# utcsilab/score-based-channels

Measured on AMD Instinct MI355X. Metric: channels/s full ALD inference, CDL-C Nt64xNr16, higher is better.
Workload: dtype f16x2 (every fp32 operand as two fp16 terms of a power-of-two-scaled value = 22-bit significand, hh + hl + lh on the fp16 matrix cores, fp32 accumulate; fp32-class by the gate tests/test_gpu_parity.py::test_f16x2_is_fp32_class and held to every reference golden at the north_star tolerance; unconditi

## Files before the change

score_based_channels_amd/csrc/conv_down.hip:

```cpp
#include <stdlib.h>
#include <string.h>
#include <type_traits>
#include "conv_common.h"

namespace sbc {

typedef float f32x4v __attribute__((ext_vector_type(4)));

struct DownParams {
    const float* __restrict__ a;
    const float* __restrict__ x;
    float* __restrict__ out;
    const float* __restrict__ stats;
    const uint4* __restrict__ w4;
    const uint4* __restrict__ w2;
    const float* __restrict__ bias;
    const float* __restrict__ bias2;
    unsigned* __restrict__ range_flag;
    float* __restrict__ calib;
    int B, H;
};

template <int B_, int E_, class F>
__device__ __forceinline__ void down_static_for(F&& f) {
    if constexpr (B_ < E_) {
        f(std::integral_constant<int, B_>{});
        down_static_for<B_ + 1, E_>(f);
    }
}

template <int CIN, int COUT, int W>
__global__ __launch_bounds__(256, 2) void conv_down_kernel(DownParams p) {
    constexpr int WO = W / 2, R = 8, NR = 2 * R + 2;
    constexpr int RP = W == 16 ? 12 : 6;
    constexpr int CG = CIN / 8, KH = CIN / 32, C4 = CIN / 4, NCB = COUT / 16;
    constexpr int NU = R * WO / 16;
    constexpr int RPU = 16 / WO;
    constexpr int PS = (2 * NR * RP * 16 + 255) / 256 * 256;
    constexpr int TERM = CG * PS;
    static_assert(NCB == 4, "four waves, one 16-output-channel block each");
    static_assert((W == 16 && CIN == 32) || (W == 8 && CIN == 64), "res2.0 (32 -> 64 at 16-pixel rows) and res3.0 (64 -> 64 at 8)");
    extern __shared__ __attribute__((aligned(256))) unsigned char smem[];

    const int tid = threadIdx.x, lane = tid & 63;
    const int cb = __builtin_amdgcn_readfirstlane(tid >> 6);
    const int kq = lane >> 4, n = lane & 15;
    const int H = p.H, HO = H / 2;
    const int tiles = HO / R;
    const int s = blockIdx.x / tiles, y0 = (blockIdx.x - s * tiles) * R;
    const int r_in0 = 2 * y0 - 1;

    const int wl_base = (((kq >> 1) * (COUT / 32) + (cb >> 1)) * 2) * 64 + (16 * (cb & 1) + n) + 32 * (kq & 1);
    constexpr int WD = 4;
    uint4 wr[WD][2];
    auto ldw = [&](const uint4* __restrict__ w, int tap, int kh, int slot) {
        const int idx = wl_base + ((tap * (CIN / 16) + 2 * kh) * (COUT / 32) * 2) * 64;
        wr[slot][0] = w[idx];
        wr[slot][1] = w[idx + 64];
    };
    const float4 tr4 = f16x2_trailer(reinterpret_cast<const float4*>(p.w4), 16 * (CIN / 16) * (COUT / 32) * 2);
    const float4 tr2 = f16x2_trailer(reinterpret_cast<const float4*>(p.w2), 4 * (CIN / 16) * (COUT / 32) * 2);
    const float scale_m = __builtin_bit_cast(float, __builtin_amdgcn_readfirstlane(__builtin_bit_cast(int, tr4.x)));
    const float scale_s = __builtin_bit_cast(float, __builtin_amdgcn_readfirstlane(__builtin_bit_cast(int, tr2.x)));
    const float descale_m = tr4.y, descale_s = tr2.y;
    const bool elu_acc = __builtin_amdgcn_readfirstlane(__builtin_bit_cast(int, tr4.w)) != 0;
    unsigned rbits = 0;

    const int c4 = tid % C4;
    constexpr int CPR = W * C4;
    auto plane_dst = [&](int prow, int col) {
        return smem + (c4 >> 1) * PS + (((col & 1) * NR + prow) * RP + (col >> 1) + (col & 1)) * 16 + (c4 & 1) * 8;
    };
    for (int i = tid; i < 2 * TERM / 16; i += 256) *reinterpret_cast<uint4*>(smem + i * 16) = make_uint4(0, 0, 0, 0);

    constexpr int NQA = NR * CPR / 256, NQX = 2 * R * CPR / 256;
    static_assert(NR * CPR % 256 == 0 && 2 * R * CPR % 256 == 0, "whole rounds of chunks");
    float4 va[NQA];
    const float* a_base = p.a + (size_t)s * H * W * CIN;
#pragma unroll
    for (int k = 0; k < NQA; ++k) {
        const int q = k * 256 + tid, prow = q / CPR;
        const int r = r_in0 + prow;
        va[k] = make_float4(0.f, 0.f, 0.f, 0.f);
        if (r >= 0 && r < H) va[k] = *reinterpret_cast<const float4*>(a_base + (size_t)r * W * CIN + (q - prow * CPR) * 4);
    }
    const float* st = p.stats + (size_t)s * 3 * CIN + c4 * 4;
    const float4 mu = *reinterpret_cast<const float4*>(st), sc = *reinterpret_cast<const float4*>(st + CIN),
                 sh = *reinterpret_cast<const float4*>(st + 2 * CIN);
    ldw(p.w4, 0, 0, 0);
    ldw(p.w4, 1 / KH, 1 % KH, 1);
    ldw(p.w4, 2 / KH, 2 % KH, 2);
    __syncthreads();
    float ta = 0.f;
#pragma unroll
    for (int k = 0; k < NQA; ++k) {
        const int q = k * 256 + tid, prow = q / CPR, col = (q - prow * CPR) / C4;
        const int r = r_in0 + prow;
        if (r < 0 || r >= H) continue;
        float4 v = va[k];
        v.x = fmaf(v.x - mu.x, sc.x, sh.x); v.y = fmaf(v.y - mu.y, sc.y, sh.y);
        v.z = fmaf(v.z - mu.z, sc.z, sh.z); v.w = fmaf(v.w - mu.w, sc.w, sh.w);
        v = elu4(v, elu_acc);
        StageScale ss{scale_m, ta};
        scale_track(v, &ss);
        ta = ss.amax;
        uint2 h, l;
        split_f16x2(v, scale_m, h, l);
        unsigned char* dst = plane_dst(prow, col);
        *reinterpret_cast<uint2*>(dst) = h;
        *reinterpret_cast<uint2*>(dst + TERM) = l;
    }
    pair_range_tile(ta, scale_m, rbits, p.calib);
    float4 vx[NQX];
    const float* x_base = p.x + ((size_t)s * H + 2 * y0) * W * CIN;
#pragma unroll
    for (int k = 0; k < NQX; ++k) vx[k] = *reinterpret_cast<const float4*>(x_base + (size_t)(k * 256 + tid) * 4);
    lds_barrier();

    const int yl0 = n / WO, xo = n % WO;
    const int rd_base = kq * PS + ((2 * yl0) * RP + xo) * 16;
    f32x4v accm[NU], accs[NU];
    auto kloop = [&](auto mainc, const uint4* __restrict__ w, f32x4v* acc) {
        constexpr bool MAIN = decltype(mainc)::value;
        constexpr int KT = MAIN ? 4 : 2, NS = KT * KT * KH;
        down_static_for<0, NS>([&](auto sc_) {
            constexpr int s_ = decltype(sc_)::value;
            constexpr int tap = s_ / KH, kh = s_ % KH, tp = tap / KT, tq = tap % KT;
            if constexpr (s_ + WD - 1 < NS) ldw(w, (s_ + WD - 1) / KH, (s_ + WD - 1) % KH, (s_ + WD - 1) % WD);
            const f16x8 wh = __builtin_bit_cast(f16x8, wr[s_ % WD][0]);
            const f16x8 wl = __builtin_bit_cast(f16x8, wr[s_ % WD][1]);
            constexpr int prow = MAIN ? tp : tp + 1, q = MAIN ? tq : tq + 1;
            constexpr int off = (4 * kh) * PS + ((((q + 1) & 1) * NR + prow) * RP + (q >> 1)) * 16;
            f16x8 xh[NU], xl[NU];
#pragma unroll
            for (int u = 0; u < NU; ++u) {
                xh[u] = *reinterpret_cast<const f16x8*>(smem + rd_base + off + (2 * u * RPU * RP) * 16);
                xl[u] = *reinterpret_cast<const f16x8*>(smem + rd_base + off + (2 * u * RPU * RP) * 16 + TERM);
            }
#pragma unroll
            for (int u = 0; u < NU; ++u) {
                const f32x4v z = s_ == 0 ? f32x4v{0.f, 0.f, 0.f, 0.f} : acc[u];
                acc[u] = __builtin_amdgcn_mfma_f32_16x16x32_f16(wh, xl[u], z, 0, 0, 0);
            }
#pragma unroll
            for (int u = 0; u < NU; ++u) acc[u] = __builtin_amdgcn_mfma_f32_16x16x32_f16(wl, xh[u], acc[u], 0, 0, 0);
#pragma unroll
            for (int u = 0; u < NU; ++u) acc[u] = __builtin_amdgcn_mfma_f32_16x16x32_f16(wh, xh[u], acc[u], 0, 0, 0);
            __builtin_amdgcn_sched_barrier(0);
        });
    };
    kloop(std::true_type{}, p.w4, accm);

    ldw(p.w2, 0, 0, 0);
    ldw(p.w2, 1 / KH, 1 % KH, 1);
    ldw(p.w2, 2 / KH, 2 % KH, 2);
    float tb = 0.f;
    uint2 xh_[NQX], xl_[NQX];
#pragma unroll
    for (int k = 0; k < NQX; ++k) {
        StageScale ss{scale_s, tb};
        scale_track(vx[k], &ss);
        tb = ss.amax;
        split_f16x2(vx[k], scale_s, xh_[k], xl_[k]);
    }
    pair_range_tile(tb, scale_s, rbits, p.calib ? p.calib + 1 : nullptr);
    lds_barrier();
#pragma unroll
    for (int k = 0; k < NQX; ++k) {
        const int q = k * 256 + tid, prow = q / CPR, col = (q - prow * CPR) / C4;
        unsigned char* dst = plane_dst(prow + 1, col);
        *reinterpret_cast<uint2*>(dst) = xh_[k];
        *reinterpret_cast<uint2*>(dst + TERM) = xl_[k];
    }
    lds_barrier();
    kloop(std::false_type{}, p.w2, accs);

    const int ch0 = 16 * cb + 4 * kq;
    const f32x4v b2 = *reinterpret_cast<const f32x4v*>(p.bias + ch0), bs = *reinterpret_cast<const f32x4v*>(p.bias2 + ch0);
#pragma unroll
    for (int u = 0; u < NU; ++u) {
        float4 o;
        o.x = fmaf(accs[u][0], descale_s, bs[0]) + fmaf(accm[u][0], descale_m, b2[0]);
        o.y = fmaf(accs[u][1], descale_s, bs[1]) + fmaf(accm[u][1], descale_m, b2[1]);
        o.z = fmaf(accs[u][2], descale_s, bs[2]) + fmaf(accm[u][2], descale_m, b2[2]);
        o.w = fmaf(accs[u][3], descale_s, bs[3]) + fmaf(accm[u][3], descale_m, b2[3]);
        const int y = y0 + u * RPU + yl0;
        st_out(p.out + (((size_t)s * HO + y) * WO + xo) * COUT + ch0, o);
    }
    if (rbits && lane == 0) atomicOr(p.range_flag, rbits);
}

template <int CIN, int COUT, int W>
static int launch_down_t(const DownParams& p, hipStream_t stream, bool dry) {
    constexpr int NR = 18, RP = W == 16 ? 12 : 6;
    constexpr int PS = (2 * NR * RP * 16 + 255) / 256 * 256;
    constexpr int LDS = 2 * (CIN / 8) * PS;
    auto kern = conv_down_kernel<CIN, COUT, W>;
    { const int rc = ensure_dyn_lds(reinterpret_cast<const void*>(kern), LDS); if (rc) return rc; }
    if (dry) return SBC_OK;
    hipLaunchKernelGGL(kern, dim3(p.B * (p.H / 2 / 8)), dim3(256), LDS, stream, p);
    SBC_CHECK_HIP(hipGetLastError());
    return SBC_OK;
}

int launch_conv_down(const sbc_op& op, hipStream_t stream, bool dry) {
    SBC_REQUIRE(op.in && op.out && op.res1 && op.stats && op.weight_split && op.weight2_split && op.bias && op.bias2,
                "conv_down: in / res1 / out / stats / weight_split / weight2_split / bias / bias2 must be set");
    SBC_REQUIRE((op.W == 16 && op.cin == 32 && op.cout == 64) || (op.W == 8 && op.cin == 64 && op.cout == 64),
                "conv_down: 32 -> 64 channels at 16-pixel rows or 64 -> 64 at 8 (got %d -> %d, W = %d)", op.cin, op.cout, op.W);
    SBC_REQUIRE(op.H % 16 == 0 && op.H >= 16, "conv_down: H = %d must be a multiple of 16 (tiles of 8 pooled rows)", op.H);
    SBC_REQUIRE((op.flags & SBC_CONV_F16X2) && !(op.flags & SBC_CONV_F16W), "conv_down: SBC_CONV_F16X2 only (the weight forms it reads)");
    SBC_REQUIRE(op.out != op.in && op.out != op.res1, "conv_down: out must not alias its inputs");
    SBC_REQUIRE(op.B > 0 && (long)op.B * op.H * op.W * op.cin <= 0x7fffffffL, "conv_down: bad batch %d", op.B);
    DownParams p;
    memset(&p, 0, sizeof(p));
    p.a = (const float*)op.in; p.x = (const float*)op.res1; p.out = (float*)op.out; p.stats = (const float*)op.stats;
    p.w4 = (const uint4*)op.weight_split; p.w2 = (const uint4*)op.weight2_split;
    p.bias = (const float*)op.bias; p.bias2 = (const float*)op.bias2;
    p.calib = (float*)op.calib;
    p.B = op.B; p.H = op.H;
    unsigned* flag = nullptr;
    { const int rc = range_flag_ptr(&flag); if (rc) return rc; }
    p.range_flag = flag;
    return op.W == 16 ? launch_down_t<32, 64, 16>(p, stream, dry) : launch_down_t<64, 64, 8>(p, stream, dry);
}

}
```

score_based_channels_amd/csrc/conv_res.hip:

```cpp
#include <type_traits>
#include "conv_common.h"

namespace sbc {

typedef float f32x4v __attribute__((ext_vector_type(4)));

struct ResParams {
    const float* __restrict__ in;
    float* __restrict__ out;
    const uint4* __restrict__ w1;
    const uint4* __restrict__ w2;
    const float* __restrict__ bias1;
    const float* __restrict__ bias2;
    const float* __restrict__ stats1;
    const float* __restrict__ norm2;
    float* __restrict__ pm_out;
    unsigned* __restrict__ range_flag;
    float* __restrict__ calib;
    int B;
    unsigned long long tail_pad;
};

__device__ __forceinline__ float row_sum16(float v) {
    v += __builtin_bit_cast(float, __builtin_amdgcn_update_dpp(0, __builtin_bit_cast(int, v), 0x128 , 0xf, 0xf, false));
    v += __builtin_bit_cast(float, __builtin_amdgcn_update_dpp(0, __builtin_bit_cast(int, v), 0x124 , 0xf, 0xf, false));
    v += __builtin_bit_cast(float, __builtin_amdgcn_update_dpp(0, __builtin_bit_cast(int, v), 0x122 , 0xf, 0xf, false));
    v += __builtin_bit_cast(float, __builtin_amdgcn_update_dpp(0, __builtin_bit_cast(int, v), 0x121 , 0xf, 0xf, false));
    return v;
}

__global__ __launch_bounds__(512, 2) void conv_res_kernel(ResParams p) {
    constexpr int C = 32, W = 16, H = 64, NT = 2, KGS = C / 8;
    constexpr int WP = W + 2, PR = H + 2;
    constexpr int PS = (PR * WP * 16 + 255) / 256 * 256;
    constexpr int RED_OFF = NT * KGS * PS;
    constexpr int MV_OFF = RED_OFF + 8 * C * 2 * 4;
    constexpr int NRM_OFF = MV_OFF + 2 * C * 4;
    constexpr int NU = 16;
    extern __shared__ __attribute__((aligned(256))) unsigned char smem[];

    const int tid = threadIdx.x, lane = tid & 63;
    const int wave = __builtin_amdgcn_readfirstlane(tid >> 6);
    const int hf = wave & 1, sub = wave >> 1;
    const int kq = lane >> 4, c = lane & 15;
    const int cq = 4 * hf + kq;

    constexpr int WD = 4;
    static_assert(WD % 2 == 0, "an odd ring depth makes hipcc merge the two K loops into one loop over a scratch-resident ring");
    uint4 wr[WD][NT];
    const uint4* wb = nullptr;
    auto ldw = [&](int tap) {
#pragma unroll
        for (int t = 0; t < NT; ++t) wr[tap % WD][t] = wb[(tap * (C / 16) * NT + t) * 64];
    };
    auto load_w = [&](const uint4* __restrict__ w) {
        int lo = lane;
        asm volatile("" : "+v"(lo));
        wb = w + ((lo >> 5) * NT) * 64 + (16 * hf + (lo & 15)) + 32 * ((lo >> 4) & 1);
#pragma unroll
        for (int tap = 0; tap < WD - 1; ++tap) ldw(tap);
    };
    const float4 t1 = f16x2_trailer(reinterpret_cast<const float4*>(p.w1), 9 * (C / 16) * (C / 32) * NT);
    const float4 t2 = f16x2_trailer(reinterpret_cast<const float4*>(p.w2), 9 * (C / 16) * (C / 32) * NT);
    const float scale1 = __builtin_bit_cast(float, __builtin_amdgcn_readfirstlane(__builtin_bit_cast(int, t1.x)));
    const float scale2 = __builtin_bit_cast(float, __builtin_amdgcn_readfirstlane(__builtin_bit_cast(int, t2.x)));
    const float descale1 = t1.y, descale2 = t2.y;
    const float4 b1 = *reinterpret_cast<const float4*>(p.bias1 + cq * 4), b2 = *reinterpret_cast<const float4*>(p.bias2 + cq * 4);
    float al = 0.f, ga = 0.f, be = 0.f;
    if (tid < C) { al = p.norm2[tid]; ga = p.norm2[C + tid]; be = p.norm2[2 * C + tid]; }
    unsigned rbits = 0;
    if (t1.w != 0.f || t2.w != 0.f) rbits |= 4u;

    for (int i = tid; i < NT * KGS * PS / 16; i += 512) *reinterpret_cast<uint4*>(smem + i * 16) = make_uint4(0, 0, 0, 0);

    float4 xr[NU], mu, sc, sh;
    auto request_x = [&](int n) {
        int lo = lane;
        asm volatile("" : "+v"(lo));
        const float* src = p.in + (size_t)(((n * H + sub * NU) * W + (lo & 15)) * C + (4 * hf + (lo >> 4)) * 4);
#pragma unroll
        for (int i = 0; i < NU; ++i) xr[i] = *reinterpret_cast<const float4*>(src + i * W * C);
        const float* st = p.stats1 + (size_t)n * 3 * C + (4 * hf + (lo >> 4)) * 4;
        mu = *reinterpret_cast<const float4*>(st); sc = *reinterpret_cast<const float4*>(st + C); sh = *reinterpret_cast<const float4*>(st + 2 * C);
    };
    int n = blockIdx.x;
    if (n < p.B) request_x(n);
    load_w(p.w1);

    for (; n < p.B; n += gridDim.x) {
        __syncthreads();
        int lq = lane;
        asm volatile("" : "+v"(lq));
        unsigned char* const dst0 = smem + ((4 * hf + (lq >> 4)) >> 1) * PS + ((sub * NU + 1) * WP + (lq & 15) + 1) * 16 + ((lq >> 4) & 1) * 8;
        float ta = 0.f, tb = 0.f;
#pragma unroll
        for (int i = 0; i < NU; ++i) {
            float4 v = make_float4(fmaf(xr[i].x - mu.x, sc.x, sh.x), fmaf(xr[i].y - mu.y, sc.y, sh.y),
                                   fmaf(xr[i].z - mu.z, sc.z, sh.z), fmaf(xr[i].w - mu.w, sc.w, sh.w));
            v = elu4(v);
            StageScale ss{scale1, ta};
            scale_track(v, &ss);
            ta = ss.amax;
            uint2 h, l;
            split_f16x2(v, scale1, h, l);
            *reinterpret_cast<uint2*>(dst0 + i * WP * 16) = h;
            *reinterpret_cast<uint2*>(dst0 + i * WP * 16 + KGS * PS) = l;
        }
        pair_range_tile(ta, scale1, rbits, p.calib);
        lds_barrier();

        f32x4v acc[NU];
        auto conv = [&]() __attribute__((always_inline)) {
            int ub[NT];
            ub[0] = kq * PS + ((sub * NU) * WP + c) * 16;
#pragma unroll
            for (int t = 1; t < NT; ++t) { ub[t] = ub[0] + t * KGS * PS; asm volatile("" : "+v"(ub[t])); }
            constexpr int NS = 9 * NU, D = 3;
            f16x8 ring[D][NT];
            auto ld = [&](int s) {
                const int tap = s / NU, i = s % NU;
                const int off = ((i + tap / 3) * WP + (tap % 3)) * 16;
#pragma unroll
                for (int t = 0; t < NT; ++t) ring[s % D][t] = *reinterpret_cast<const f16x8*>(smem + ub[t] + off);
            };
#pragma unroll
            for (int s = 0; s < D - 1; ++s) ld(s);
            __builtin_amdgcn_s_setprio(3);
#pragma unroll
            for (int s = 0; s < NS; ++s) {
                const int tap = s / NU, i = s % NU;
                if (s + D - 1 < NS) ld(s + D - 1);
                if (i == 0 && tap + WD - 1 < 9) ldw(tap + WD - 1);
                const f16x8 xh = ring[s % D][0], xl = ring[s % D][1];
                const f16x8 wh = __builtin_bit_cast(f16x8, wr[tap % WD][0]), wl = __builtin_bit_cast(f16x8, wr[tap % WD][1]);
                const f32x4v c0 = tap == 0 ? f32x4v{0.f, 0.f, 0.f, 0.f} : acc[i];
                acc[i] = __builtin_amdgcn_mfma_f32_16x16x32_f16(wh, xl, c0, 0, 0, 0);
                acc[i] = __builtin_amdgcn_mfma_f32_16x16x32_f16(wl, xh, acc[i], 0, 0, 0);
                acc[i] = __builtin_amdgcn_mfma_f32_16x16x32_f16(wh, xh, acc[i], 0, 0, 0);
                __builtin_amdgcn_sched_barrier(0);
            }
            __builtin_amdgcn_s_setprio(0);
        };
        auto tile_moments = [&](int T, float (&mean)[4], float (&m2)[4]) {
#pragma unroll
            for (int r = 0; r < 4; ++r) {
                float s = 0.f;
#pragma unroll
                for (int i = 0; i < 8; ++i) s += acc[8 * T + i][r];
                mean[r] = row_sum16(s) * (1.f / 128.f);
                float q = 0.f;
#pragma unroll
                for (int i = 0; i < 8; ++i) { const float d = acc[8 * T + i][r] - mean[r]; q = fmaf(d, d, q); }
                m2[r] = row_sum16(q);
            }
        };

        conv();
        load_w(p.w2);
        {
#pragma unroll
            for (int i = 0; i < NU; ++i) {
                acc[i][0] = fmaf(acc[i][0], descale1, b1.x); acc[i][1] = fmaf(acc[i][1], descale1, b1.y);
                acc[i][2] = fmaf(acc[i][2], descale1, b1.z); acc[i][3] = fmaf(acc[i][3], descale1, b1.w);
            }
        }
        float* red = reinterpret_cast<float*>(smem + RED_OFF);
        float* mv = reinterpret_cast<float*>(smem + MV_OFF);
        float* nrm = reinterpret_cast<float*>(smem + NRM_OFF);
#pragma unroll
        for (int T = 0; T < 2; ++T) {
            float mean[4], m2[4];
            tile_moments(T, mean, m2);
            if (c == 0) {
#pragma unroll
                for (int r = 0; r < 4; ++r)
                    *reinterpret_cast<float2*>(red + ((2 * sub + T) * C + cq * 4 + r) * 2) = make_float2(mean[r], m2[r]);
            }
        }
        lds_barrier();
        if (tid < C) {
            float mw[8], m_c = 0.f, q = 0.f;
#pragma unroll
            for (int t = 0; t < 8; ++t) { const float2 v = *reinterpret_cast<const float2*>(red + (t * C + tid) * 2); mw[t] = v.x; m_c += v.x; q += v.y; }
            m_c *= 0.125f;
            float dd = 0.f;
#pragma unroll
            for (int t = 0; t < 8; ++t) { const float d = mw[t] - m_c; dd = fmaf(d, d, dd); }
            const float var_c = fmaf(128.f, dd, q) * (1.f / (float)(H * W));
            mv[tid] = m_c;
            asm volatile("s_waitcnt lgkmcnt(0)" ::: "memory");
            float m = 0.f;
#pragma unroll
            for (int k = 0; k < C; k += 4) { const float4 v = *reinterpret_cast<const float4*>(mv + k); m += v.x; m += v.y; m += v.z; m += v.w; }
            m *= 1.f / (float)C;
            float v = 0.f;
#pragma unroll
            for (int k = 0; k < C; k += 4) {
                const float4 u = *reinterpret_cast<const float4*>(mv + k);
                float d = u.x - m; v = fmaf(d, d, v);
                d = u.y - m; v = fmaf(d, d, v);
                d = u.z - m; v = fmaf(d, d, v);
                d = u.w - m; v = fmaf(d, d, v);
            }
            v *= 1.f / (float)(C - 1);
            const float rs = 1.f / sqrtf(v + 1e-5f);
            nrm[tid] = m_c;
            nrm[C + tid] = ga / sqrtf(fmaxf(var_c, 0.f) + 1e-5f);
            nrm[2 * C + tid] = fmaf(ga, (m_c - m) * rs * al, be);
        }
        lds_barrier();
        const float4 nmu = *reinterpret_cast<const float4*>(nrm + cq * 4), nsc = *reinterpret_cast<const float4*>(nrm + C + cq * 4),
                     nsh = *reinterpret_cast<const float4*>(nrm + 2 * C + cq * 4);
#pragma unroll
        for (int i = 0; i < NU; ++i) {
            float4 v = make_float4(fmaf(acc[i][0] - nmu.x, nsc.x, nsh.x), fmaf(acc[i][1] - nmu.y, nsc.y, nsh.y),
                                   fmaf(acc[i][2] - nmu.z, nsc.z, nsh.z), fmaf(acc[i][3] - nmu.w, nsc.w, nsh.w));
            v = elu4(v);
            StageScale ss{scale2, tb};
            scale_track(v, &ss);
            tb = ss.amax;
            uint2 h, l;
            split_f16x2(v, scale2, h, l);
            *reinterpret_cast<uint2*>(dst0 + i * WP * 16) = h;
            *reinterpret_cast<uint2*>(dst0 + i * WP * 16 + KGS * PS) = l;
        }
        pair_range_tile(tb, scale2, rbits, p.calib ? p.calib + 1 : nullptr);
        lds_barrier();
        conv();
        load_w(p.w1);
#pragma unroll
        for (int i = 0; i < NU; ++i) {
            acc[i][0] = fmaf(acc[i][0], descale2, b2.x) + xr[i].x; acc[i][1] = fmaf(acc[i][1], descale2, b2.y) + xr[i].y;
            acc[i][2] = fmaf(acc[i][2], descale2, b2.z) + xr[i].z; acc[i][3] = fmaf(acc[i][3], descale2, b2.w) + xr[i].w;
        }
        __builtin_amdgcn_sched_barrier(0);
        request_x(min(n + (int)gridDim.x, p.B - 1));
        __builtin_amdgcn_sched_barrier(0);
        {
            float* const o = p.out + (size_t)(((n * H + sub * NU) * W + (lq & 15)) * C + (4 * hf + (lq >> 4)) * 4);
#pragma unroll
            for (int i = 0; i < NU; ++i) st_out(o + i * W * C, make_float4(acc[i][0], acc[i][1], acc[i][2], acc[i][3]));
        }
        if (p.pm_out) {
#pragma unroll
            for (int T = 0; T < 2; ++T) {
                float mean[4], m2[4];
                tile_moments(T, mean, m2);
                if (c == 0) {
#pragma unroll
                    for (int r = 0; r < 4; ++r)
                        *reinterpret_cast<float2*>(p.pm_out + (((size_t)n * 8 + 2 * sub + T) * C + cq * 4 + r) * 2) = make_float2(mean[r], m2[r]);
                }
            }
        }
    }
    if (rbits && lane == 0) atomicOr(p.range_flag, rbits);
}

int launch_res_block(const sbc_op& op, hipStream_t stream, bool dry) {
    SBC_REQUIRE(op.in && op.out && op.weight_split && op.weight2_split && op.bias && op.bias2 && op.stats && op.norm2,
                "res_block: in / out / weight_split / weight2_split / bias / bias2 / stats / norm2 must be set");
    SBC_REQUIRE(op.cin == 32 && op.cout == 32 && op.ksize == 3 && op.dil == 1 && op.H == 64 && op.W == 16,
                "res_block: 32 -> 32 -> 32 channels, 3x3, undilated, 64 x 16 samples (got %d -> %d, %dx%d)", op.cin, op.cout, op.H, op.W);
    SBC_REQUIRE(op.B > 0, "res_block: bad batch %d", op.B);
    SBC_REQUIRE(op.out != op.in, "res_block: out must not alias in (the next sample is requested while the epilogue stores)");
    SBC_REQUIRE((op.flags & SBC_CONV_F16X2) && !(op.flags & SBC_CONV_F16W), "res_block: SBC_CONV_F16X2 only (the weight forms it reads)");
    SBC_REQUIRE(!(op.flags & SBC_EPI_MOMENTS_OUT) || op.aux, "res_block: SBC_EPI_MOMENTS_OUT without aux");
    SBC_REQUIRE(!(op.flags & (SBC_EPI_POOL | SBC_EPI_UP | SBC_EPI_ELUGRAD | SBC_EPI_RES1_ELU)) && !op.res1 && !op.res2 && !op.up,
                "res_block: the residual operand is the input itself; no other epilogue");
    SBC_REQUIRE((long)op.B * op.H * op.W * op.cin <= 0x7fffffffL, "res_block: tensor exceeds the 32-bit element index");
    constexpr size_t lds = (size_t)2 * 4 * ((66 * 18 * 16 + 255) / 256 * 256) + 8 * 32 * 2 * 4 + 2 * 32 * 4 + 3 * 32 * 4;
    static_assert(lds <= 160 * 1024, "LDS of the one resident workgroup");
    { const int rc = ensure_dyn_lds(reinterpret_cast<const void*>(conv_res_kernel), lds); if (rc) return rc; }
    unsigned* word = nullptr;
    { const int rc = range_flag_ptr(&word); if (rc) return rc; }
    if (dry) return SBC_OK;
    ResParams p{};
    p.in = (const float*)op.in; p.out = (float*)op.out;
    p.w1 = (const uint4*)op.weight_split; p.w2 = (const uint4*)op.weight2_split;
    p.bias1 = (const float*)op.bias; p.bias2 = (const float*)op.bias2;
    p.stats1 = (const float*)op.stats; p.norm2 = (const float*)op.norm2;
    p.pm_out = (op.flags & SBC_EPI_MOMENTS_OUT) ? (float*)op.aux : nullptr;
    p.range_flag = word; p.calib = (float*)op.calib; p.B = op.B;
    int dev = 0, cus = 256;
    SBC_CHECK_HIP(hipGetDevice(&dev));
    SBC_CHECK_HIP(hipDeviceGetAttribute(&cus, hipDeviceAttributeMultiprocessorCount, dev));
    hipLaunchKernelGGL(conv_res_kernel, dim3(balanced_sample_grid(op.B, cus)), dim3(512), lds, stream, p);
    SBC_CHECK_HIP(hipGetLastError());
    return SBC_OK;
}

}
```

Baseline: 56.47.

## Make conv_down persistent with cross-tile prefetch of activations and filters

Turns the down-sampling conv kernel into a persistent kernel: the grid is capped at two blocks per CU and each block walks a contiguous range of tiles. Activations, residual input and the first filter slices for the next tile are requested during the current tile's MFMA loops, using a deeper filter ring that spans both the main and shortcut filters. LDS operand reads are double-buffered one step ahead of the MFMAs. This hides global-load latency and launch/tail cost, at the price of more registers, a zeroed LDS halo rewritten per tile, and a host device-attribute query on every launch.

```diff
diff --git a/score_based_channels_amd/csrc/conv_down.hip b/score_based_channels_amd/csrc/conv_down.hip
--- a/score_based_channels_amd/csrc/conv_down.hip
+++ b/score_based_channels_amd/csrc/conv_down.hip
@@ -46,17 +46,30 @@
     const int cb = __builtin_amdgcn_readfirstlane(tid >> 6);
     const int kq = lane >> 4, n = lane & 15;
     const int H = p.H, HO = H / 2;
-    const int tiles = HO / R;
-    const int s = blockIdx.x / tiles, y0 = (blockIdx.x - s * tiles) * R;
-    const int r_in0 = 2 * y0 - 1;
-
-    const int wl_base = (((kq >> 1) * (COUT / 32) + (cb >> 1)) * 2) * 64 + (16 * (cb & 1) + n) + 32 * (kq & 1);
-    constexpr int WD = 4;
+    const int tiles = HO / R, ntiles = p.B * tiles;
+    const int t_begin = (int)((long)blockIdx.x * ntiles / gridDim.x), t_end = (int)((long)(blockIdx.x + 1) * ntiles / gridDim.x);
+
+    constexpr int NSM = 16 * KH, NSS = 4 * KH, NTOT = NSM + NSS;
+#ifndef DOWN_WD2
+#define DOWN_WD2 9
+#endif
+#ifndef DOWN_WD4
+#define DOWN_WD4 6
+#endif
+    constexpr int WD = NU <= 2 ? DOWN_WD2 : DOWN_WD4;
+    constexpr int PF = NTOT - WD;
+    static_assert(WD > NSS && PF >= 0, "the ring holds the whole shortcut filter: no filter request behind the main K loop");
+    int wl_base = (((kq >> 1) * (COUT / 32) + (cb >> 1)) * 2) * 64 + (16 * (cb & 1) + n) + 32 * (kq & 1);
     uint4 wr[WD][2];
     auto ldw = [&](const uint4* __restrict__ w, int tap, int kh, int slot) {
         const int idx = wl_base + ((tap * (CIN / 16) + 2 * kh) * (COUT / 32) * 2) * 64;
         wr[slot][0] = w[idx];
         wr[slot][1] = w[idx + 64];
+    };
+    auto ldg = [&](auto gc) {
+        constexpr int g = decltype(gc)::value;
+        if constexpr (g < NSM) ldw(p.w4, g / KH, g % KH, g % WD);
+        else ldw(p.w2, (g - NSM) / KH, (g - NSM) % KH, g % WD);
     };
     const float4 tr4 = f16x2_trailer(reinterpret_cast<const float4*>(p.w4), 16 * (CIN / 16) * (COUT / 32) * 2);
     const float4 tr2 = f16x2_trailer(reinterpret_cast<const float4*>(p.w2), 4 * (CIN / 16) * (COUT / 32) * 2);
@@ -71,121 +84,166 @@
     auto plane_dst = [&](int prow, int col) {
         return smem + (c4 >> 1) * PS + (((col & 1) * NR + prow) * RP + (col >> 1) + (col & 1)) * 16 + (c4 & 1) * 8;
     };
-    for (int i = tid; i < 2 * TERM / 16; i += 256) *reinterpret_cast<uint4*>(smem + i * 16) = make_uint4(0, 0, 0, 0);
-
     constexpr int NQA = NR * CPR / 256, NQX = 2 * R * CPR / 256;
     static_assert(NR * CPR % 256 == 0 && 2 * R * CPR % 256 == 0, "whole rounds of chunks");
-    float4 va[NQA];
-    const float* a_base = p.a + (size_t)s * H * W * CIN;
-#pragma unroll
-    for (int k = 0; k < NQA; ++k) {
-        const int q = k * 256 + tid, prow = q / CPR;
-        const int r = r_in0 + prow;
-        va[k] = make_float4(0.f, 0.f, 0.f, 0.f);
-        if (r >= 0 && r < H) va[k] = *reinterpret_cast<const float4*>(a_base + (size_t)r * W * CIN + (q - prow * CPR) * 4);
+    static_assert(CPR == 128, "a round of chunks is two rows: only the first and the last round touch a halo row");
+    float4 va[NQA], vx[NQX], mu, sc, sh;
+    auto req_a = [&](int tile) {
+        const int s = tile / tiles, y0 = (tile - s * tiles) * R;
+        const float* base = p.a + ((size_t)s * H + 2 * y0) * W * CIN - W * CIN + tid * 4;
+#pragma unroll
+        for (int k = 0; k < NQA; ++k) {
+            const float* src = base + k * 1024;
+            if (k == 0 && y0 == 0 && tid < CPR) src += W * CIN;
+            if (k == NQA - 1 && y0 + R == HO && tid >= CPR) src -= W * CIN;
+            va[k] = *reinterpret_cast<const float4*>(src);
+        }
+        const float* st = p.stats + (size_t)s * 3 * CIN + c4 * 4;
+        mu = *reinterpret_cast<const float4*>(st);
+        sc = *reinterpret_cast<const float4*>(st + CIN);
+        sh = *reinterpret_cast<const float4*>(st + 2 * CIN);
+    };
+    auto req_x = [&](int tile) {
+        const int s = tile / tiles, y0 = (tile - s * tiles) * R;
+        const float* base = p.x + ((size_t)s * H + 2 * y0) * W * CIN + tid * 4;
+#pragma unroll
+        for (int k = 0; k < NQX; ++k) vx[k] = *reinterpret_cast<const float4*>(base + k * 1024);
+    };
+    if (t_begin < t_end) {
+        req_a(t_begin);
+        __builtin_amdgcn_sched_barrier(0);
+        req_x(t_begin);
+        __builtin_amdgcn_sched_barrier(0);
+        down_static_for<0, WD - 1>([&](auto gc) { ldg(gc); });
+        __builtin_amdgcn_sched_barrier(0);
     }
-    const float* st = p.stats + (size_t)s * 3 * CIN + c4 * 4;
-    const float4 mu = *reinterpret_cast<const float4*>(st), sc = *reinterpret_cast<const float4*>(st + CIN),
-                 sh = *reinterpret_cast<const float4*>(st + 2 * CIN);
-    ldw(p.w4, 0, 0, 0);
-    ldw(p.w4, 1 / KH, 1 % KH, 1);
-    ldw(p.w4, 2 / KH, 2 % KH, 2);
-    __syncthreads();
-    float ta = 0.f;
-#pragma unroll
-    for (int k = 0; k < NQA; ++k) {
-        const int q = k * 256 + tid, prow = q / CPR, col = (q - prow * CPR) / C4;
-        const int r = r_in0 + prow;
-        if (r < 0 || r >= H) continue;
-        float4 v = va[k];
-        v.x = fmaf(v.x - mu.x, sc.x, sh.x); v.y = fmaf(v.y - mu.y, sc.y, sh.y);
-        v.z = fmaf(v.z - mu.z, sc.z, sh.z); v.w = fmaf(v.w - mu.w, sc.w, sh.w);
-        v = elu4(v, elu_acc);
-        StageScale ss{scale_m, ta};
-        scale_track(v, &ss);
-        ta = ss.amax;
-        uint2 h, l;
-        split_f16x2(v, scale_m, h, l);
-        unsigned char* dst = plane_dst(prow, col);
-        *reinterpret_cast<uint2*>(dst) = h;
-        *reinterpret_cast<uint2*>(dst + TERM) = l;
-    }
-    pair_range_tile(ta, scale_m, rbits, p.calib);
-    float4 vx[NQX];
-    const float* x_base = p.x + ((size_t)s * H + 2 * y0) * W * CIN;
-#pragma unroll
-    for (int k = 0; k < NQX; ++k) vx[k] = *reinterpret_cast<const float4*>(x_base + (size_t)(k * 256 + tid) * 4);
-    lds_barrier();
+    for (int i = tid; i < 2 * TERM / 16; i += 256) *reinterpret_cast<uint4*>(smem + i * 16) = make_uint4(0, 0, 0, 0);
 
     const int yl0 = n / WO, xo = n % WO;
     const int rd_base = kq * PS + ((2 * yl0) * RP + xo) * 16;
+    const int ch0 = 16 * cb + 4 * kq;
+    const f32x4v b2 = *reinterpret_cast<const f32x4v*>(p.bias + ch0), bs = *reinterpret_cast<const f32x4v*>(p.bias2 + ch0);
     f32x4v accm[NU], accs[NU];
-    auto kloop = [&](auto mainc, const uint4* __restrict__ w, f32x4v* acc) {
+#ifndef DOWN_XLATE
+#define DOWN_XLATE 0
+#endif
+#ifndef DOWN_XRING
+#define DOWN_XRING 1
+#endif
+    constexpr int XB = DOWN_XRING ? 1 : 0;
+    f16x8 xh[XB + 1][NU], xl[XB + 1][NU];
+    int tn = t_begin;
+    auto ldx = [&](auto mainc, auto sc_) {
         constexpr bool MAIN = decltype(mainc)::value;
-        constexpr int KT = MAIN ? 4 : 2, NS = KT * KT * KH;
+        constexpr int KT = MAIN ? 4 : 2;
+        constexpr int s_ = decltype(sc_)::value, tap = s_ / KH, kh = s_ % KH, tp = tap / KT, tq = tap % KT;
+        constexpr int prow = MAIN ? tp : tp + 1, q = MAIN ? tq : tq + 1;
+        constexpr int off = (4 * kh) * PS + ((((q + 1) & 1) * NR + prow) * RP + (q >> 1)) * 16;
+#pragma unroll
+        for (int u = 0; u < NU; ++u) {
+            xh[s_ & XB][u] = *reinterpret_cast<const f16x8*>(smem + rd_base + off + (2 * u * RPU * RP) * 16);
+            xl[s_ & XB][u] = *reinterpret_cast<const f16x8*>(smem + rd_base + off + (2 * u * RPU * RP) * 16 + TERM);
+        }
+    };
+    auto kloop = [&](auto mainc, f32x4v* acc) {
+        constexpr bool MAIN = decltype(mainc)::value;
+        constexpr int NS = MAIN ? NSM : NSS, G0 = MAIN ? 0 : NSM;
+        if constexpr (XB) ldx(mainc, std::integral_constant<int, 0>{});
         down_static_for<0, NS>([&](auto sc_) {
-            constexpr int s_ = decltype(sc_)::value;
-            constexpr int tap = s_ / KH, kh = s_ % KH, tp = tap / KT, tq = tap % KT;
-            if constexpr (s_ + WD - 1 < NS) ldw(w, (s_ + WD - 1) / KH, (s_ + WD - 1) % KH, (s_ + WD - 1) % WD);
-            const f16x8 wh = __builtin_bit_cast(f16x8, wr[s_ % WD][0]);
-            const f16x8 wl = __builtin_bit_cast(f16x8, wr[s_ % WD][1]);
-            constexpr int prow = MAIN ? tp : tp + 1, q = MAIN ? tq : tq + 1;
-            constexpr int off = (4 * kh) * PS + ((((q + 1) & 1) * NR + prow) * RP + (q >> 1)) * 16;
-            f16x8 xh[NU], xl[NU];
-#pragma unroll
-            for (int u = 0; u < NU; ++u) {
-                xh[u] = *reinterpret_cast<const f16x8*>(smem + rd_base + off + (2 * u * RPU * RP) * 16);
-                xl[u] = *reinterpret_cast<const f16x8*>(smem + rd_base + off + (2 * u * RPU * RP) * 16 + TERM);
-            }
+            constexpr int s_ = decltype(sc_)::value, g = G0 + s_;
+            if constexpr (g + WD - 1 < NTOT) ldg(std::integral_constant<int, g + WD - 1>{});
+            if constexpr (g == PF) req_a(tn);
+            if constexpr (!XB) ldx(mainc, sc_);
+            else if constexpr (s_ + 1 < NS) ldx(mainc, std::integral_constant<int, s_ + 1>{});
+            const f16x8 wh = __builtin_bit_cast(f16x8, wr[g % WD][0]);
+            const f16x8 wl = __builtin_bit_cast(f16x8, wr[g % WD][1]);
 #pragma unroll
             for (int u = 0; u < NU; ++u) {
                 const f32x4v z = s_ == 0 ? f32x4v{0.f, 0.f, 0.f, 0.f} : acc[u];
-                acc[u] = __builtin_amdgcn_mfma_f32_16x16x32_f16(wh, xl[u], z, 0, 0, 0);
+                acc[u] = __builtin_amdgcn_mfma_f32_16x16x32_f16(wh, xl[s_ & XB][u], z, 0, 0, 0);
             }
 #pragma unroll
-            for (int u = 0; u < NU; ++u) acc[u] = __builtin_amdgcn_mfma_f32_16x16x32_f16(wl, xh[u], acc[u], 0, 0, 0);
-#pragma unroll
-            for (int u = 0; u < NU; ++u) acc[u] = __builtin_amdgcn_mfma_f32_16x16x32_f16(wh, xh[u], acc[u], 0, 0, 0);
+            for (int u = 0; u < NU; ++u) acc[u] = __builtin_amdgcn_mfma_f32_16x16x32_f16(wl, xh[s_ & XB][u], acc[u], 0, 0, 0);
+#pragma unroll
+            for (int u = 0; u < NU; ++u) acc[u] = __builtin_amdgcn_mfma_f32_16x16x32_f16(wh, xh[s_ & XB][u], acc[u], 0, 0, 0);
             __builtin_amdgcn_sched_barrier(0);
         });
     };
-    kloop(std::true_type{}, p.w4, accm);
-
-    ldw(p.w2, 0, 0, 0);
-    ldw(p.w2, 1 / KH, 1 % KH, 1);
-    ldw(p.w2, 2 / KH, 2 % KH, 2);
-    float tb = 0.f;
-    uint2 xh_[NQX], xl_[NQX];
-#pragma unroll
-    for (int k = 0; k < NQX; ++k) {
-        StageScale ss{scale_s, tb};
-        scale_track(vx[k], &ss);
-        tb = ss.amax;
-        split_f16x2(vx[k], scale_s, xh_[k], xl_[k]);
-    }
-    pair_range_tile(tb, scale_s, rbits, p.calib ? p.calib + 1 : nullptr);
-    lds_barrier();
-#pragma unroll
-    for (int k = 0; k < NQX; ++k) {
-        const int q = k * 256 + tid, prow = q / CPR, col = (q - prow * CPR) / C4;
-        unsigned char* dst = plane_dst(prow + 1, col);
-        *reinterpret_cast<uint2*>(dst) = xh_[k];
-        *reinterpret_cast<uint2*>(dst + TERM) = xl_[k];
-    }
-    lds_barrier();
-    kloop(std::false_type{}, p.w2, accs);
-
-    const int ch0 = 16 * cb + 4 * kq;
-    const f32x4v b2 = *reinterpret_cast<const f32x4v*>(p.bias + ch0), bs = *reinterpret_cast<const f32x4v*>(p.bias2 + ch0);
-#pragma unroll
-    for (int u = 0; u < NU; ++u) {
-        float4 o;
-        o.x = fmaf(accs[u][0], descale_s, bs[0]) + fmaf(accm[u][0], descale_m, b2[0]);
-        o.y = fmaf(accs[u][1], descale_s, bs[1]) + fmaf(accm[u][1], descale_m, b2[1]);
-        o.z = fmaf(accs[u][2], descale_s, bs[2]) + fmaf(accm[u][2], descale_m, b2[2]);
-        o.w = fmaf(accs[u][3], descale_s, bs[3]) + fmaf(accm[u][3], descale_m, b2[3]);
-        const int y = y0 + u * RPU + yl0;
-        st_out(p.out + (((size_t)s * HO + y) * WO + xo) * COUT + ch0, o);
+
+#pragma unroll 1
+    for (int tile = t_begin; tile < t_end; ++tile) {
+        const int s = tile / tiles, y0 = (tile - s * tiles) * R;
+        tn = min(tile + 1, t_end - 1);
+        asm volatile("" : "+v"(wl_base));
+        lds_barrier();
+
+        float ta = 0.f;
+#pragma unroll
+        for (int k = 0; k < NQA; ++k) {
+            const int q = k * 256 + tid, prow = q / CPR, col = (q - prow * CPR) / C4;
+            unsigned char* dst = plane_dst(prow, col);
+            uint2 h = make_uint2(0, 0), l = make_uint2(0, 0);
+            const bool outside = (k == 0 && y0 == 0 && prow == 0) || (k == NQA - 1 && y0 + R == HO && prow == NR - 1);
+            if (!outside) {
+                float4 v = va[k];
+                v.x = fmaf(v.x - mu.x, sc.x, sh.x); v.y = fmaf(v.y - mu.y, sc.y, sh.y);
+                v.z = fmaf(v.z - mu.z, sc.z, sh.z); v.w = fmaf(v.w - mu.w, sc.w, sh.w);
+                v = elu4(v, elu_acc);
+                StageScale ss{scale_m, ta};
+                scale_track(v, &ss);
+                ta = ss.amax;
+                split_f16x2(v, scale_m, h, l);
+            }
+            *reinterpret_cast<uint2*>(dst) = h;
+            *reinterpret_cast<uint2*>(dst + TERM) = l;
+        }
+        pair_range_tile(ta, scale_m, rbits, p.calib);
+        lds_barrier();
+        kloop(std::true_type{}, accm);
+
+        float tb = 0.f;
+        uint2 xh_[NQX], xl_[NQX];
+#pragma unroll
+        for (int k = 0; k < NQX; ++k) {
+            StageScale ss{scale_s, tb};
+            scale_track(vx[k], &ss);
+            tb = ss.amax;
+            split_f16x2(vx[k], scale_s, xh_[k], xl_[k]);
+        }
+#if DOWN_XLATE == 0
+        __builtin_amdgcn_sched_barrier(0);
+        req_x(tn);
+        __builtin_amdgcn_sched_barrier(0);
+#endif
+        pair_range_tile(tb, scale_s, rbits, p.calib ? p.calib + 1 : nullptr);
+        lds_barrier();
+#pragma unroll
+        for (int k = 0; k < NQX; ++k) {
+            const int q = k * 256 + tid, prow = q / CPR, col = (q - prow * CPR) / C4;
+            unsigned char* dst = plane_dst(prow + 1, col);
+            *reinterpret_cast<uint2*>(dst) = xh_[k];
+            *reinterpret_cast<uint2*>(dst + TERM) = xl_[k];
+        }
+        lds_barrier();
+        kloop(std::false_type{}, accs);
+        __builtin_amdgcn_sched_barrier(0);
+#if DOWN_XLATE
+        req_x(tn);
+        __builtin_amdgcn_sched_barrier(0);
+#endif
+        down_static_for<0, WD - 1>([&](auto gc) { ldg(gc); });
+        __builtin_amdgcn_sched_barrier(0);
+
+#pragma unroll
+        for (int u = 0; u < NU; ++u) {
+            float4 o;
+            o.x = fmaf(accs[u][0], descale_s, bs[0]) + fmaf(accm[u][0], descale_m, b2[0]);
+            o.y = fmaf(accs[u][1], descale_s, bs[1]) + fmaf(accm[u][1], descale_m, b2[1]);
+            o.z = fmaf(accs[u][2], descale_s, bs[2]) + fmaf(accm[u][2], descale_m, b2[2]);
+            o.w = fmaf(accs[u][3], descale_s, bs[3]) + fmaf(accm[u][3], descale_m, b2[3]);
+            const int y = y0 + u * RPU + yl0;
+            st_out(p.out + (((size_t)s * HO + y) * WO + xo) * COUT + ch0, o);
+        }
     }
     if (rbits && lane == 0) atomicOr(p.range_flag, rbits);
 }
@@ -198,7 +256,16 @@
     auto kern = conv_down_kernel<CIN, COUT, W>;
     { const int rc = ensure_dyn_lds(reinterpret_cast<const void*>(kern), LDS); if (rc) return rc; }
     if (dry) return SBC_OK;
-    hipLaunchKernelGGL(kern, dim3(p.B * (p.H / 2 / 8)), dim3(256), LDS, stream, p);
+    int dev = 0, cus = 256;
+    SBC_CHECK_HIP(hipGetDevice(&dev));
+    SBC_CHECK_HIP(hipDeviceGetAttribute(&cus, hipDeviceAttributeMultiprocessorCount, dev));
+    const int ntiles = p.B * (p.H / 2 / 8);
+#ifdef DOWN_GRID_ALL
+    const int grid = ntiles;
+#else
+    const int grid = max(1, min(ntiles, 2 * persistent_cus(cus)));
+#endif
+    hipLaunchKernelGGL(kern, dim3(grid), dim3(256), LDS, stream, p);
     SBC_CHECK_HIP(hipGetLastError());
     return SBC_OK;
 }
```

Result: no change. 56.49, median of 3 (+0.0%).

## Give each wave both output-channel halves over eight rows in residual block kernel

Applied to the files above, without the earlier changes.

The work split changes. Before, each wave held one 16-channel half for 16 rows. Now each wave computes all 32 output channels for 8 rows, so every input-fragment LDS read feeds two MFMA groups instead of one, halving activation LDS traffic per MFMA. In exchange the weight registers per wave double. Bias and norm parameters move from per-thread registers into LDS to ease register pressure, at the cost of extra LDS reads in the epilogues.

```diff
diff --git a/score_based_channels_amd/csrc/conv_res.hip b/score_based_channels_amd/csrc/conv_res.hip
--- a/score_based_channels_amd/csrc/conv_res.hip
+++ b/score_based_channels_amd/csrc/conv_res.hip
@@ -18,7 +18,6 @@
     unsigned* __restrict__ range_flag;
     float* __restrict__ calib;
     int B;
-    unsigned long long tail_pad;
 };
 
 __device__ __forceinline__ float row_sum16(float v) {
@@ -30,33 +29,34 @@
 }
 
 __global__ __launch_bounds__(512, 2) void conv_res_kernel(ResParams p) {
-    constexpr int C = 32, W = 16, H = 64, NT = 2, KGS = C / 8;
+    constexpr int C = 32, W = 16, H = 64, NT = 2, KGS = C / 8, NB = C / 16;
     constexpr int WP = W + 2, PR = H + 2;
     constexpr int PS = (PR * WP * 16 + 255) / 256 * 256;
     constexpr int RED_OFF = NT * KGS * PS;
     constexpr int MV_OFF = RED_OFF + 8 * C * 2 * 4;
     constexpr int NRM_OFF = MV_OFF + 2 * C * 4;
-    constexpr int NU = 16;
+    constexpr int PRM_OFF = NRM_OFF + 3 * C * 4;
+    constexpr int NU = 8;
     extern __shared__ __attribute__((aligned(256))) unsigned char smem[];
 
     const int tid = threadIdx.x, lane = tid & 63;
     const int wave = __builtin_amdgcn_readfirstlane(tid >> 6);
-    const int hf = wave & 1, sub = wave >> 1;
     const int kq = lane >> 4, c = lane & 15;
-    const int cq = 4 * hf + kq;
 
     constexpr int WD = 4;
     static_assert(WD % 2 == 0, "an odd ring depth makes hipcc merge the two K loops into one loop over a scratch-resident ring");
-    uint4 wr[WD][NT];
+    uint4 wr[WD][NB][NT];
     const uint4* wb = nullptr;
     auto ldw = [&](int tap) {
 #pragma unroll
-        for (int t = 0; t < NT; ++t) wr[tap % WD][t] = wb[(tap * (C / 16) * NT + t) * 64];
+        for (int j = 0; j < NB; ++j)
+#pragma unroll
+            for (int t = 0; t < NT; ++t) wr[tap % WD][j][t] = wb[(tap * (C / 16) * NT + t) * 64 + 16 * j];
     };
     auto load_w = [&](const uint4* __restrict__ w) {
         int lo = lane;
         asm volatile("" : "+v"(lo));
-        wb = w + ((lo >> 5) * NT) * 64 + (16 * hf + (lo & 15)) + 32 * ((lo >> 4) & 1);
+        wb = w + ((lo >> 5) * NT) * 64 + (lo & 15) + 32 * ((lo >> 4) & 1);
 #pragma unroll
         for (int tap = 0; tap < WD - 1; ++tap) ldw(tap);
     };
@@ -64,24 +64,34 @@
     const float4 t2 = f16x2_trailer(reinterpret_cast<const float4*>(p.w2), 9 * (C / 16) * (C / 32) * NT);
     const float scale1 = __builtin_bit_cast(float, __builtin_amdgcn_readfirstlane(__builtin_bit_cast(int, t1.x)));
     const float scale2 = __builtin_bit_cast(float, __builtin_amdgcn_readfirstlane(__builtin_bit_cast(int, t2.x)));
-    const float descale1 = t1.y, descale2 = t2.y;
-    const float4 b1 = *reinterpret_cast<const float4*>(p.bias1 + cq * 4), b2 = *reinterpret_cast<const float4*>(p.bias2 + cq * 4);
-    float al = 0.f, ga = 0.f, be = 0.f;
-    if (tid < C) { al = p.norm2[tid]; ga = p.norm2[C + tid]; be = p.norm2[2 * C + tid]; }
+    const float descale1 = __builtin_bit_cast(float, __builtin_amdgcn_readfirstlane(__builtin_bit_cast(int, t1.y)));
+    const float descale2 = __builtin_bit_cast(float, __builtin_amdgcn_readfirstlane(__builtin_bit_cast(int, t2.y)));
+    if (tid < C) {
+        float* prm0 = reinterpret_cast<float*>(smem + PRM_OFF);
+        prm0[tid] = p.bias1[tid]; prm0[C + tid] = p.bias2[tid];
+        prm0[2 * C + tid] = p.norm2[tid]; prm0[3 * C + tid] = p.norm2[C + tid]; prm0[4 * C + tid] = p.norm2[2 * C + tid];
+    }
+    auto fresh_tid = [&]() { int t = tid; asm volatile("" : "+v"(t)); return t; };
     unsigned rbits = 0;
     if (t1.w != 0.f || t2.w != 0.f) rbits |= 4u;
 
     for (int i = tid; i < NT * KGS * PS / 16; i += 512) *reinterpret_cast<uint4*>(smem + i * 16) = make_uint4(0, 0, 0, 0);
 
-    float4 xr[NU], mu, sc, sh;
+    float4 xr[NU][NB], mu[NB], sc[NB], sh[NB];
     auto request_x = [&](int n) {
         int lo = lane;
         asm volatile("" : "+v"(lo));
-        const float* src = p.in + (size_t)(((n * H + sub * NU) * W + (lo & 15)) * C + (4 * hf + (lo >> 4)) * 4);
-#pragma unroll
-        for (int i = 0; i < NU; ++i) xr[i] = *reinterpret_cast<const float4*>(src + i * W * C);
-        const float* st = p.stats1 + (size_t)n * 3 * C + (4 * hf + (lo >> 4)) * 4;
-        mu = *reinterpret_cast<const float4*>(st); sc = *reinterpret_cast<const float4*>(st + C); sh = *reinterpret_cast<const float4*>(st + 2 * C);
+        const float* src = p.in + (size_t)(((n * H + wave * NU) * W + (lo & 15)) * C + (lo >> 4) * 4);
+#pragma unroll
+        for (int i = 0; i < NU; ++i)
+#pragma unroll
+            for (int j = 0; j < NB; ++j) xr[i][j] = *reinterpret_cast<const float4*>(src + i * W * C + 16 * j);
+        const float* st = p.stats1 + (size_t)n * 3 * C + (lo >> 4) * 4;
+#pragma unroll
+        for (int j = 0; j < NB; ++j) {
+            mu[j] = *reinterpret_cast<const float4*>(st + 16 * j); sc[j] = *reinterpret_cast<const float4*>(st + C + 16 * j);
+            sh[j] = *reinterpret_cast<const float4*>(st + 2 * C + 16 * j);
+        }
     };
     int n = blockIdx.x;
     if (n < p.B) request_x(n);
@@ -91,28 +101,32 @@
         __syncthreads();
         int lq = lane;
         asm volatile("" : "+v"(lq));
-        unsigned char* const dst0 = smem + ((4 * hf + (lq >> 4)) >> 1) * PS + ((sub * NU + 1) * WP + (lq & 15) + 1) * 16 + ((lq >> 4) & 1) * 8;
+        unsigned char* const dst0 = smem + (lq >> 5) * PS + ((wave * NU + 1) * WP + (lq & 15) + 1) * 16 + ((lq >> 4) & 1) * 8;
         float ta = 0.f, tb = 0.f;
 #pragma unroll
-        for (int i = 0; i < NU; ++i) {
-            float4 v = make_float4(fmaf(xr[i].x - mu.x, sc.x, sh.x), fmaf(xr[i].y - mu.y, sc.y, sh.y),
-                                   fmaf(xr[i].z - mu.z, sc.z, sh.z), fmaf(xr[i].w - mu.w, sc.w, sh.w));
-            v = elu4(v);
-            StageScale ss{scale1, ta};
-            scale_track(v, &ss);
-            ta = ss.amax;
-            uint2 h, l;
-            split_f16x2(v, scale1, h, l);
-            *reinterpret_cast<uint2*>(dst0 + i * WP * 16) = h;
-            *reinterpret_cast<uint2*>(dst0 + i * WP * 16 + KGS * PS) = l;
+        for (int j = 0; j < NB; ++j) {
+#pragma unroll
+            for (int i = 0; i < NU; ++i) {
+                const float4 x = xr[i][j];
+                float4 v = make_float4(fmaf(x.x - mu[j].x, sc[j].x, sh[j].x), fmaf(x.y - mu[j].y, sc[j].y, sh[j].y),
+                                       fmaf(x.z - mu[j].z, sc[j].z, sh[j].z), fmaf(x.w - mu[j].w, sc[j].w, sh[j].w));
+                v = elu4(v);
+                StageScale ss{scale1, ta};
+                scale_track(v, &ss);
+                ta = ss.amax;
+                uint2 h, l;
+                split_f16x2(v, scale1, h, l);
+                *reinterpret_cast<uint2*>(dst0 + 2 * j * PS + i * WP * 16) = h;
+                *reinterpret_cast<uint2*>(dst0 + 2 * j * PS + i * WP * 16 + KGS * PS) = l;
+            }
         }
         pair_range_tile(ta, scale1, rbits, p.calib);
         lds_barrier();
 
-        f32x4v acc[NU];
+        f32x4v acc[NU][NB];
         auto conv = [&]() __attribute__((always_inline)) {
             int ub[NT];
-            ub[0] = kq * PS + ((sub * NU) * WP + c) * 16;
+            ub[0] = kq * PS + ((wave * NU) * WP + c) * 16;
 #pragma unroll
             for (int t = 1; t < NT; ++t) { ub[t] = ub[0] + t * KGS * PS; asm volatile("" : "+v"(ub[t])); }
             constexpr int NS = 9 * NU, D = 3;
@@ -132,62 +146,68 @@
                 if (s + D - 1 < NS) ld(s + D - 1);
                 if (i == 0 && tap + WD - 1 < 9) ldw(tap + WD - 1);
                 const f16x8 xh = ring[s % D][0], xl = ring[s % D][1];
-                const f16x8 wh = __builtin_bit_cast(f16x8, wr[tap % WD][0]), wl = __builtin_bit_cast(f16x8, wr[tap % WD][1]);
-                const f32x4v c0 = tap == 0 ? f32x4v{0.f, 0.f, 0.f, 0.f} : acc[i];
-                acc[i] = __builtin_amdgcn_mfma_f32_16x16x32_f16(wh, xl, c0, 0, 0, 0);
-                acc[i] = __builtin_amdgcn_mfma_f32_16x16x32_f16(wl, xh, acc[i], 0, 0, 0);
-                acc[i] = __builtin_amdgcn_mfma_f32_16x16x32_f16(wh, xh, acc[i], 0, 0, 0);
+#pragma unroll
+                for (int j = 0; j < NB; ++j) {
+                    const f16x8 wh = __builtin_bit_cast(f16x8, wr[tap % WD][j][0]), wl = __builtin_bit_cast(f16x8, wr[tap % WD][j][1]);
+                    const f32x4v c0 = tap == 0 ? f32x4v{0.f, 0.f, 0.f, 0.f} : acc[i][j];
+                    acc[i][j] = __builtin_amdgcn_mfma_f32_16x16x32_f16(wh, xl, c0, 0, 0, 0);
+                    acc[i][j] = __builtin_amdgcn_mfma_f32_16x16x32_f16(wl, xh, acc[i][j], 0, 0, 0);
+                    acc[i][j] = __builtin_amdgcn_mfma_f32_16x16x32_f16(wh, xh, acc[i][j], 0, 0, 0);
+                }
                 __builtin_amdgcn_sched_barrier(0);
             }
             __builtin_amdgcn_s_setprio(0);
         };
-        auto tile_moments = [&](int T, float (&mean)[4], float (&m2)[4]) {
+        auto tile_moments = [&](int j, float (&mean)[4], float (&m2)[4]) {
 #pragma unroll
             for (int r = 0; r < 4; ++r) {
                 float s = 0.f;
 #pragma unroll
-                for (int i = 0; i < 8; ++i) s += acc[8 * T + i][r];
+                for (int i = 0; i < NU; ++i) s += acc[i][j][r];
                 mean[r] = row_sum16(s) * (1.f / 128.f);
                 float q = 0.f;
 #pragma unroll
-                for (int i = 0; i < 8; ++i) { const float d = acc[8 * T + i][r] - mean[r]; q = fmaf(d, d, q); }
+                for (int i = 0; i < NU; ++i) { const float d = acc[i][j][r] - mean[r]; q = fmaf(d, d, q); }
                 m2[r] = row_sum16(q);
             }
         };
 
         conv();
         load_w(p.w2);
-        {
-#pragma unroll
-            for (int i = 0; i < NU; ++i) {
-                acc[i][0] = fmaf(acc[i][0], descale1, b1.x); acc[i][1] = fmaf(acc[i][1], descale1, b1.y);
-                acc[i][2] = fmaf(acc[i][2], descale1, b1.z); acc[i][3] = fmaf(acc[i][3], descale1, b1.w);
-            }
-        }
         float* red = reinterpret_cast<float*>(smem + RED_OFF);
         float* mv = reinterpret_cast<float*>(smem + MV_OFF);
         float* nrm = reinterpret_cast<float*>(smem + NRM_OFF);
-#pragma unroll
-        for (int T = 0; T < 2; ++T) {
+        const float* prm = reinterpret_cast<const float*>(smem + PRM_OFF);
+        const int kqc = (fresh_tid() >> 4) & 3;
+#pragma unroll
+        for (int j = 0; j < NB; ++j) {
+            const float4 b1 = *reinterpret_cast<const float4*>(prm + (4 * j + kqc) * 4);
+#pragma unroll
+            for (int i = 0; i < NU; ++i) {
+                acc[i][j][0] = fmaf(acc[i][j][0], descale1, b1.x); acc[i][j][1] = fmaf(acc[i][j][1], descale1, b1.y);
+                acc[i][j][2] = fmaf(acc[i][j][2], descale1, b1.z); acc[i][j][3] = fmaf(acc[i][j][3], descale1, b1.w);
+            }
             float mean[4], m2[4];
-            tile_moments(T, mean, m2);
+            tile_moments(j, mean, m2);
             if (c == 0) {
 #pragma unroll
                 for (int r = 0; r < 4; ++r)
-                    *reinterpret_cast<float2*>(red + ((2 * sub + T) * C + cq * 4 + r) * 2) = make_float2(mean[r], m2[r]);
+                    *reinterpret_cast<float2*>(red + (wave * C + (4 * j + kqc) * 4 + r) * 2) = make_float2(mean[r], m2[r]);
             }
         }
         lds_barrier();
         if (tid < C) {
+            const int ch = fresh_tid();
+            const float al = prm[2 * C + ch], ga = prm[3 * C + ch], be = prm[4 * C + ch];
             float mw[8], m_c = 0.f, q = 0.f;
 #pragma unroll
-            for (int t = 0; t < 8; ++t) { const float2 v = *reinterpret_cast<const float2*>(red + (t * C + tid) * 2); mw[t] = v.x; m_c += v.x; q += v.y; }
+            for (int t = 0; t < 8; ++t) { const float2 v = *reinterpret_cast<const float2*>(red + (t * C + ch) * 2); mw[t] = v.x; m_c += v.x; q += v.y; }
             m_c *= 0.125f;
             float dd = 0.f;
 #pragma unroll
             for (int t = 0; t < 8; ++t) { const float d = mw[t] - m_c; dd = fmaf(d, d, dd); }
             const float var_c = fmaf(128.f, dd, q) * (1.f / (float)(H * W));
-            mv[tid] = m_c;
+            mv[ch] = m_c;
             asm volatile("s_waitcnt lgkmcnt(0)" ::: "memory");
             float m = 0.f;
 #pragma unroll
@@ -204,52 +224,66 @@
             }
             v *= 1.f / (float)(C - 1);
             const float rs = 1.f / sqrtf(v + 1e-5f);
-            nrm[tid] = m_c;
-            nrm[C + tid] = ga / sqrtf(fmaxf(var_c, 0.f) + 1e-5f);
-            nrm[2 * C + tid] = fmaf(ga, (m_c - m) * rs * al, be);
+            nrm[ch] = m_c;
+            nrm[C + ch] = ga / sqrtf(fmaxf(var_c, 0.f) + 1e-5f);
+            nrm[2 * C + ch] = fmaf(ga, (m_c - m) * rs * al, be);
         }
         lds_barrier();
-        const float4 nmu = *reinterpret_cast<const float4*>(nrm + cq * 4), nsc = *reinterpret_cast<const float4*>(nrm + C + cq * 4),
-                     nsh = *reinterpret_cast<const float4*>(nrm + 2 * C + cq * 4);
-#pragma unroll
-        for (int i = 0; i < NU; ++i) {
-            float4 v = make_float4(fmaf(acc[i][0] - nmu.x, nsc.x, nsh.x), fmaf(acc[i][1] - nmu.y, nsc.y, nsh.y),
-                                   fmaf(acc[i][2] - nmu.z, nsc.z, nsh.z), fmaf(acc[i][3] - nmu.w, nsc.w, nsh.w));
-            v = elu4(v);
-            StageScale ss{scale2, tb};
-            scale_track(v, &ss);
-            tb = ss.amax;
-            uint2 h, l;
-            split_f16x2(v, scale2, h, l);
-            *reinterpret_cast<uint2*>(dst0 + i * WP * 16) = h;
-            *reinterpret_cast<uint2*>(dst0 + i * WP * 16 + KGS * PS) = l;
+        const int kqd = (fresh_tid() >> 4) & 3;
+#pragma unroll
+        for (int j = 0; j < NB; ++j) {
+            const int cq = 4 * j + kqd;
+            const float4 nmu = *reinterpret_cast<const float4*>(nrm + cq * 4), nsc = *reinterpret_cast<const float4*>(nrm + C + cq * 4),
+                         nsh = *reinterpret_cast<const float4*>(nrm + 2 * C + cq * 4);
+#pragma unroll
+            for (int i = 0; i < NU; ++i) {
+                float4 v = make_float4(fmaf(acc[i][j][0] - nmu.x, nsc.x, nsh.x), fmaf(acc[i][j][1] - nmu.y, nsc.y, nsh.y),
+                                       fmaf(acc[i][j][2] - nmu.z, nsc.z, nsh.z), fmaf(acc[i][j][3] - nmu.w, nsc.w, nsh.w));
+                v = elu4(v);
+                StageScale ss{scale2, tb};
+                scale_track(v, &ss);
+                tb = ss.amax;
+                uint2 h, l;
+                split_f16x2(v, scale2, h, l);
+                *reinterpret_cast<uint2*>(dst0 + 2 * j * PS + i * WP * 16) = h;
+                *reinterpret_cast<uint2*>(dst0 + 2 * j * PS + i * WP * 16 + KGS * PS) = l;
+            }
         }
         pair_range_tile(tb, scale2, rbits, p.calib ? p.calib + 1 : nullptr);
         lds_barrier();
         conv();
         load_w(p.w1);
-#pragma unroll
-        for (int i = 0; i < NU; ++i) {
-            acc[i][0] = fmaf(acc[i][0], descale2, b2.x) + xr[i].x; acc[i][1] = fmaf(acc[i][1], descale2, b2.y) + xr[i].y;
-            acc[i][2] = fmaf(acc[i][2], descale2, b2.z) + xr[i].z; acc[i][3] = fmaf(acc[i][3], descale2, b2.w) + xr[i].w;
+        const int kqf = (fresh_tid() >> 4) & 3;
+#pragma unroll
+        for (int j = 0; j < NB; ++j) {
+            const float4 b2 = *reinterpret_cast<const float4*>(prm + C + (4 * j + kqf) * 4);
+#pragma unroll
+            for (int i = 0; i < NU; ++i) {
+                acc[i][j][0] = fmaf(acc[i][j][0], descale2, b2.x) + xr[i][j].x; acc[i][j][1] = fmaf(acc[i][j][1], descale2, b2.y) + xr[i][j].y;
+                acc[i][j][2] = fmaf(acc[i][j][2], descale2, b2.z) + xr[i][j].z; acc[i][j][3] = fmaf(acc[i][j][3], descale2, b2.w) + xr[i][j].w;
+            }
         }
         __builtin_amdgcn_sched_barrier(0);
         request_x(min(n + (int)gridDim.x, p.B - 1));
         __builtin_amdgcn_sched_barrier(0);
         {
-            float* const o = p.out + (size_t)(((n * H + sub * NU) * W + (lq & 15)) * C + (4 * hf + (lq >> 4)) * 4);
-#pragma unroll
-            for (int i = 0; i < NU; ++i) st_out(o + i * W * C, make_float4(acc[i][0], acc[i][1], acc[i][2], acc[i][3]));
+            const int lf = fresh_tid();
+            float* const o = p.out + (size_t)(((n * H + wave * NU) * W + (lf & 15)) * C + ((lf >> 4) & 3) * 4);
+#pragma unroll
+            for (int i = 0; i < NU; ++i)
+#pragma unroll
+                for (int j = 0; j < NB; ++j)
+                    st_out(o + i * W * C + 16 * j, make_float4(acc[i][j][0], acc[i][j][1], acc[i][j][2], acc[i][j][3]));
         }
         if (p.pm_out) {
 #pragma unroll
-            for (int T = 0; T < 2; ++T) {
+            for (int j = 0; j < NB; ++j) {
                 float mean[4], m2[4];
-                tile_moments(T, mean, m2);
+                tile_moments(j, mean, m2);
                 if (c == 0) {
 #pragma unroll
                     for (int r = 0; r < 4; ++r)
-                        *reinterpret_cast<float2*>(p.pm_out + (((size_t)n * 8 + 2 * sub + T) * C + cq * 4 + r) * 2) = make_float2(mean[r], m2[r]);
+                        *reinterpret_cast<float2*>(p.pm_out + (((size_t)n * 8 + wave) * C + (4 * j + kqf) * 4 + r) * 2) = make_float2(mean[r], m2[r]);
                 }
             }
         }
@@ -269,7 +303,7 @@
     SBC_REQUIRE(!(op.flags & (SBC_EPI_POOL | SBC_EPI_UP | SBC_EPI_ELUGRAD | SBC_EPI_RES1_ELU)) && !op.res1 && !op.res2 && !op.up,
                 "res_block: the residual operand is the input itself; no other epilogue");
     SBC_REQUIRE((long)op.B * op.H * op.W * op.cin <= 0x7fffffffL, "res_block: tensor exceeds the 32-bit element index");
-    constexpr size_t lds = (size_t)2 * 4 * ((66 * 18 * 16 + 255) / 256 * 256) + 8 * 32 * 2 * 4 + 2 * 32 * 4 + 3 * 32 * 4;
+    constexpr size_t lds = (size_t)2 * 4 * ((66 * 18 * 16 + 255) / 256 * 256) + 8 * 32 * 2 * 4 + 2 * 32 * 4 + 3 * 32 * 4 + 5 * 32 * 4;
     static_assert(lds <= 160 * 1024, "LDS of the one resident workgroup");
     { const int rc = ensure_dyn_lds(reinterpret_cast<const void*>(conv_res_kernel), lds); if (rc) return rc; }
     unsigned* word = nullptr;
```

Result: no change. 57.39 before, 57.26 after (median of 2 runs) (-0.2%).
